# mederrata/spmf

Measured on AMD Instinct MI355X. Metric: elbo_steps_per_sec, higher is better.
Workload: dtype f32

## Files before the change

spmf_amd/csrc/col_pass.hip:

```cpp
#include "common.h"
#include "kernels.h"

namespace spmf {

#ifndef COL_WIDE_WAVES
#define COL_WIDE_WAVES 4
#endif
#ifndef COL_GRP
#define COL_GRP 4
#endif

template <int KP>
__device__ __forceinline__ void pack_block(const double* __restrict__ dacc, float* __restrict__ tail,
                                           const double* __restrict__ det_slots) {
  if (det_slots) {
    constexpr int LEN = kDaccHead + KP;
    constexpr int SEG = 256 / (LEN <= 32 ? 32 : (LEN <= 64 ? 64 : 128));
    constexpr int W = 256 / SEG;
    __shared__ double seg_sum[SEG][W];
    const int i = threadIdx.x % W, g = threadIdx.x / W;
    const int nb = min(max((int)det_slots[0], 0), kDetMaxBlocks);
    const int per = (nb + SEG - 1) / SEG;
    double v = 0.0;
    if (i < LEN) {
      const double* sl = det_slots + kDetMeta + i;
      const int b1 = min(nb, (g + 1) * per);
      for (int b = g * per; b < b1; ++b) v += sl[(size_t)b * LEN];
    }
    seg_sum[g][i] = v;
    __syncthreads();
    if (threadIdx.x < LEN) {
      double t = 0.0;
#pragma unroll
      for (int s = 0; s < SEG; ++s) t += seg_sum[s][threadIdx.x];
      const float hi = (float)t;
      tail[2 * threadIdx.x] = hi;
      tail[2 * threadIdx.x + 1] = (float)(t - (double)hi);
    }
    return;
  }
  const int i = threadIdx.x;
  if (i < kDaccHead + KP) fold_dacc(i, dacc, tail, KP);
}

template <int KP, int LIK, int EPL, bool PACKED>
__global__ __launch_bounds__(256, EPL == 4 ? COL_WIDE_WAVES : 1) void col_pass_kernel(
    int D, int n_panels, int row_base, int blocks_per_panel,
    const int32_t* __restrict__ item_ptr, const int4* __restrict__ items,
    const int32_t* __restrict__ pc_row, const float* __restrict__ pc_val,
    const float* __restrict__ pc_gval, const float* __restrict__ Vp,
    const float* __restrict__ phi, const float* __restrict__ z, const float* __restrict__ gzs,
    float* __restrict__ gAp, float* __restrict__ gVp, float* __restrict__ gphi,
    const uint8_t* __restrict__ ctype, const int32_t* __restrict__ item_mid, int half_sel,
    int64_t Brows, int64_t acc_stride, const double* __restrict__ pack_dacc,
    float* __restrict__ pack_tail, int64_t dacc_stride, const uint32_t* __restrict__ pc_ent,
    int panel_rows, float* __restrict__ det_part, int64_t det_part_stride,
    const double* __restrict__ det_slots, int64_t det_stride) {
  static_assert(EPL == 1 || EPL == 4, "entries per lane and fetch: 1 or 4");
  static_assert(!PACKED || EPL == 4, "the packed lists are read by the wide fetch only");
  if (pack_dacc && blockIdx.x == 0) {
    pack_block<KP>(pack_dacc + (size_t)blockIdx.y * dacc_stride, pack_tail + (size_t)blockIdx.y * acc_stride,
                   det_slots ? det_slots + (size_t)blockIdx.y * det_stride : nullptr);
    return;
  }
  if (gridDim.y > 1) {
    const size_t sd = blockIdx.y;
    Vp += sd * (size_t)D * KP;
    phi += sd * (size_t)D;
    z += sd * (size_t)Brows * KP;
    gzs += sd * (size_t)Brows * KP;
    gAp += sd * (size_t)acc_stride;
    gVp += sd * (size_t)acc_stride;
    gphi += sd * (size_t)acc_stride;
  }
  constexpr int LPN = KP / 4;
  constexpr int NG = 64 / LPN;
  const GTable zt = gtable(z, Brows, KP), gt = gtable(gzs, Brows, KP);
  constexpr int GRP = EPL == 4 ? COL_GRP : (LPN < COL_GRP ? LPN : COL_GRP);
  static_assert((EPL * LPN) % GRP == 0, "a fetch is a whole number of gather groups");
  __shared__ __attribute__((aligned(16))) float stage[4][NG][2 * KP];
  const int lane = threadIdx.x & 63;
  const int sub = lane % LPN, grp = lane / LPN;
  const int bp_row = grp * LPN * 4;
  const int wid = threadIdx.x >> 6;
  const int64_t L = (int64_t)blockIdx.x - (pack_dacc ? 1 : 0);
  int p, ib;
  if (n_panels < 8) {
    p = (int)(L / blocks_per_panel);
    ib = (int)(L % blocks_per_panel);
  } else {
    const int x = (int)(L & 7);
    const int64_t q = L >> 3;
    p = 8 * (int)(q / blocks_per_panel) + x;
    ib = (int)(q % blocks_per_panel);
  }
  if (p >= n_panels) return;
  const int ilo = half_sel == 2 ? item_mid[p] : item_ptr[p];
  const int ihi = half_sel == 1 ? item_mid[p] : item_ptr[p + 1];
  const int i0 = ilo + ib * 4 * NG;
  if (i0 >= ihi) return;
  const int it = i0 + wid * NG + grp;
  const bool ok = it < ihi;
  int cur = 0, end = 0, d = 0;
  if (ok) {
    const int4 im = items[it];
    cur = im.x;
    end = im.x + im.y;
    d = im.z;
  }
  const float4 vp = ok ? gather4<LPN>(Vp, d, sub) : make_float4(0.f, 0.f, 0.f, 0.f);
  const float ph = ok ? phi[d] : 1.f;
  const bool bern = LIK == 2 || LIK == 4 || (LIK == 3 && ok && ctype[d]);
  float4 gV = make_float4(0.f, 0.f, 0.f, 0.f), gA = gV;
  float gph = 0.f;

  struct __attribute__((packed, aligned(4))) I4 { int x, y, z, w; };
  struct __attribute__((packed, aligned(4))) F4 { float x, y, z, w; };
  constexpr int FE = EPL * LPN;
  struct Raw {
    int r[EPL];
    float x[EPL], g[EPL];
    int cnt;
  };
  auto fetch_raw = [&](Raw& f) {
    f.cnt = min(FE, end - cur);
    const int e = cur + EPL * sub;
#pragma unroll
    for (int t = 0; t < EPL; ++t) {
      f.r[t] = 0;
      f.x[t] = 0.f;
      f.g[t] = 0.f;
    }
    if (EPL * sub < f.cnt) {
      if constexpr (EPL == 4) {
        if (PACKED) {
          const I4 w = *reinterpret_cast<const I4*>(reinterpret_cast<const int32_t*>(pc_ent) + e);
          f.r[0] = w.x; f.r[1] = w.y; f.r[2] = w.z; f.r[3] = w.w;
        } else {
          const I4 w = *reinterpret_cast<const I4*>(pc_row + e);
          const F4 v = *reinterpret_cast<const F4*>(pc_val + e);
          f.r[0] = w.x; f.r[1] = w.y; f.r[2] = w.z; f.r[3] = w.w;
          f.x[0] = v.x; f.x[1] = v.y; f.x[2] = v.z; f.x[3] = v.w;
        }
        if (LIK == 1 || LIK == 4) {
          const F4 v = *reinterpret_cast<const F4*>(pc_gval + e);
          f.g[0] = v.x; f.g[1] = v.y; f.g[2] = v.z; f.g[3] = v.w;
        }
      } else {
        f.r[0] = pc_row[e];
        f.x[0] = pc_val[e];
        if (LIK == 1 || LIK == 4) f.g[0] = pc_gval[e];
      }
    }
    cur += f.cnt;
  };
  const int pbase = PACKED ? p * panel_rows : -row_base;
  auto decode = [&](const Raw& f, int (&rr_)[EPL], float (&xx_)[EPL], float (&gx_)[EPL]) {
    const int left = f.cnt - EPL * sub;
#pragma unroll
    for (int t = 0; t < EPL; ++t) {
      const bool on = left > t;
      if (PACKED) {
        const uint32_t w = (uint32_t)f.r[t];
        rr_[t] = on ? (int)(w >> 16) + pbase : kPadRow;
        xx_[t] = on ? (float)(w & 0xffffu) : 0.f;
      } else {
        rr_[t] = on ? f.r[t] + pbase : kPadRow;
        xx_[t] = on ? f.x[t] : 0.f;
      }
      gx_[t] = on ? f.g[t] : 0.f;
    }
  };

  Raw fa, fb, fc;
  fetch_raw(fa);
  if (EPL == 1) fetch_raw(fb);
  while (__any(fa.cnt > 0)) {
    if (EPL == 1) fetch_raw(fc);
    else fetch_raw(fb);
    int rr0[EPL];
    float xx0[EPL], gx0[EPL];
    decode(fa, rr0, xx0, gx0);
    const int cnt0 = fa.cnt;
#pragma unroll
    for (int g0 = 0; g0 < FE; g0 += GRP) {
      if (__any(cnt0 > g0)) {
        float4 zz[GRP], gg[GRP];
        float xv[GRP], gv[GRP];
#pragma unroll
        for (int j = 0; j < GRP; ++j) {
          const int q = g0 + j;
          const int sa = bp_row + (q / EPL) * 4;
          const int b = __builtin_amdgcn_ds_bpermute(sa, rr0[q % EPL]);
          xv[j] = __int_as_float(__builtin_amdgcn_ds_bpermute(sa, __float_as_int(xx0[q % EPL])));
          gv[j] = (LIK == 1 || LIK == 4) ? __int_as_float(__builtin_amdgcn_ds_bpermute(sa, __float_as_int(gx0[q % EPL])))
                                         : xv[j];
          zz[j] = gather4<LPN>(zt, b, sub);
          gg[j] = gather4<LPN>(gt, b, sub);
        }
#pragma unroll
        for (int j = 0; j < GRP; ++j) {
          if (bern) {
            float wv = xv[j];
            if (LIK == 4) wv *= expf(fminf(group_sum<LPN>(dot4(zz[j], vp)), kYSat));
            gV = fma4(wv, zz[j], gV);
            gA = fma4(gv[j], gg[j], gA);
            gph += xv[j];
          } else {
            const float y = group_sum<LPN>(dot4(zz[j], vp));
            float ey = 1.f;
            const float r = (LIK == 1 ? expm1_dec(fminf(y, kYSat), ey) : y) + ph;
            const float xr = (r > 0.f && r < INFINITY) ? xv[j] * __builtin_amdgcn_rcpf(r)
                                                       : (xv[j] > 0.f ? 1.f : 0.f);
            gV = fma4(LIK == 1 ? xr * ey : xr, zz[j], gV);
            gA = fma4(gv[j], gg[j], gA);
            gph += xr;
          }
        }
      }
    }
    if (EPL == 1) {
      fa = fb;
      fb = fc;
    } else {
      fa = fb;
    }
  }
  if (det_part) {
    if (ok) {
      float4* dst = reinterpret_cast<float4*>(det_part + (size_t)blockIdx.y * det_part_stride +
                                              (size_t)(it - item_ptr[0]) * det_part_len(KP));
      dst[sub] = gV;
      dst[LPN + sub] = gA;
      if (sub == 0) dst[2 * LPN] = make_float4(gph, 0.f, 0.f, 0.f);
    }
    return;
  }
  float4* st4 = reinterpret_cast<float4*>(&stage[wid][grp][0]);
  st4[sub] = gV;
  st4[LPN + sub] = gA;
  __builtin_amdgcn_wave_barrier();
  const float* flat = &stage[wid][0][0];
#pragma unroll
  for (int i = 0; i < (NG * 2 * KP) / 64; ++i) {
    const int e = i * 64 + lane;
    const int c = e / (2 * KP), rem = e % (2 * KP);
    const int dd = __shfl(d, c * LPN);
    const int okc = __shfl((int)ok, c * LPN);
    const float v = flat[e];
    if (okc && v != 0.f) {
      float* dst = (rem >= KP ? gAp + (size_t)dd * KP + (rem - KP) : gVp + (size_t)dd * KP + rem);
      atomicAdd(dst, v);
    }
  }
  if (ok && sub == 0 && gph != 0.f) atomicAdd(&gphi[d], gph);
}

template <int KP>
static bool launch_col_t(const ColArgs& a, hipStream_t st) {
  constexpr int NG = 64 / (KP / 4);
  const int per_block = 4 * NG;
  const int bpp = (a.max_items_per_panel + per_block - 1) / per_block;
  if (bpp < 1) return false;
  const int64_t nt = (a.n_panels + 7) / 8;
  const int64_t nb = (a.n_panels < 8 ? (int64_t)a.n_panels * bpp : nt * bpp * 8) + (a.pack_dacc ? 1 : 0);
  const int4* items = reinterpret_cast<const int4*>(a.items);
#define SPMF_COL_ARGS                                                                            \
  dim3((unsigned)nb, a.S > 1 ? a.S : 1), dim3(256), 0, st, a.D, a.n_panels, a.row_base, bpp,   \
      a.item_ptr, items, a.pc_row, a.pc_val, a.pc_gval, a.Vp, a.phi, a.z, a.gzs, a.gAp, a.gVp, \
      a.gphi, a.ctype, a.item_mid, a.half_sel, a.B, a.acc_stride, a.pack_dacc, a.pack_tail,     \
      a.dacc_stride, a.pc_ent, a.panel_rows, a.det_part, a.det_part_stride, a.det_slots, a.det_stride
  const bool wide = a.pc_pad >= KP - 1;
  const bool packed = wide && a.pc_ent && a.panel_rows > 0 && a.panel_rows <= 65536;
#define SPMF_COL_LAUNCH(L_)                                                                        \
  do {                                                                                             \
    if (packed)                                                                                    \
      hipLaunchKernelGGL((col_pass_kernel<KP, L_, 4, true>), SPMF_COL_ARGS);                       \
    else if (wide)                                                                                 \
      hipLaunchKernelGGL((col_pass_kernel<KP, L_, 4, false>), SPMF_COL_ARGS);                      \
    else                                                                                           \
      hipLaunchKernelGGL((col_pass_kernel<KP, L_, 1, false>), SPMF_COL_ARGS);                      \
  } while (0)
  if (a.logt == 4) SPMF_COL_LAUNCH(4);
  else if (a.logt == 3) SPMF_COL_LAUNCH(3);
  else if (a.logt == 2) SPMF_COL_LAUNCH(2);
  else if (a.logt == 1) SPMF_COL_LAUNCH(1);
  else SPMF_COL_LAUNCH(0);
#undef SPMF_COL_LAUNCH
#undef SPMF_COL_ARGS
  return true;
}

template <int KP>
__global__ __launch_bounds__(256) void det_reduce_kernel(int D, int n_panels, const int32_t* __restrict__ list_first,
                                                         const int32_t* __restrict__ item_pos,
                                                         const int32_t* __restrict__ item_ptr,
                                                         const float* __restrict__ part, int64_t part_stride,
                                                         float* __restrict__ gAp, float* __restrict__ gVp,
                                                         float* __restrict__ gphi, int64_t acc_stride) {
  constexpr int LPN = KP / 4;
  const int sub = threadIdx.x % LPN;
  const int d = blockIdx.x * (256 / LPN) + threadIdx.x / LPN;
  if (d >= D) return;
  part += (size_t)blockIdx.y * part_stride;
  gAp += (size_t)blockIdx.y * acc_stride;
  gVp += (size_t)blockIdx.y * acc_stride;
  gphi += (size_t)blockIdx.y * acc_stride;
  const int it0 = item_ptr[0];
  float4 gV = make_float4(0.f, 0.f, 0.f, 0.f), gA = gV;
  float gph = 0.f;
  auto add_item = [&](int r) {
    const float4* src = reinterpret_cast<const float4*>(part + (size_t)(item_pos[r] - it0) * det_part_len(KP));
    const float4 a = src[sub], b = src[LPN + sub];
    gV.x += a.x; gV.y += a.y; gV.z += a.z; gV.w += a.w;
    gA.x += b.x; gA.y += b.y; gA.z += b.z; gA.w += b.w;
    if (sub == 0) gph += src[2 * LPN].x;
  };
  constexpr int DP = 8;
  for (int p0 = 0; p0 < n_panels; p0 += DP) {
    int r0[DP], r1[DP], jp[DP];
#pragma unroll
    for (int i = 0; i < DP; ++i) {
      const bool on = p0 + i < n_panels;
      const int32_t* lf = list_first + (size_t)(on ? p0 + i : p0) * D + d;
      r0[i] = on ? lf[0] : 0;
      r1[i] = on ? lf[1] : 0;
    }
#pragma unroll
    for (int i = 0; i < DP; ++i) jp[i] = r1[i] > r0[i] ? item_pos[r0[i]] - it0 : 0;
    float4 a[DP], b[DP];
    float g[DP];
#pragma unroll
    for (int i = 0; i < DP; ++i) {
      const float4* src = reinterpret_cast<const float4*>(part + (size_t)jp[i] * det_part_len(KP));
      const bool on = r1[i] > r0[i];
      a[i] = on ? src[sub] : make_float4(0.f, 0.f, 0.f, 0.f);
      b[i] = on ? src[LPN + sub] : make_float4(0.f, 0.f, 0.f, 0.f);
      g[i] = (on && sub == 0) ? src[2 * LPN].x : 0.f;
    }
#pragma unroll
    for (int i = 0; i < DP; ++i) {
      if (r1[i] > r0[i]) {
        gV.x += a[i].x; gV.y += a[i].y; gV.z += a[i].z; gV.w += a[i].w;
        gA.x += b[i].x; gA.y += b[i].y; gA.z += b[i].z; gA.w += b[i].w;
        if (sub == 0) gph += g[i];
        for (int r = r0[i] + 1; r < r1[i]; ++r) add_item(r);
      }
    }
  }
  reinterpret_cast<float4*>(gVp + (size_t)d * KP)[sub] = gV;
  reinterpret_cast<float4*>(gAp + (size_t)d * KP)[sub] = gA;
  if (sub == 0) gphi[d] = gph;
}

void launch_det_reduce(const DetReduceArgs& a, hipStream_t st) {
  if (a.D <= 0 || a.n_panels <= 0) return;
  with_kp<64>(a.KP, [&](auto kp) {
    constexpr int KP = decltype(kp)::value, cols = 256 / (KP / 4);
    hipLaunchKernelGGL((det_reduce_kernel<KP>), dim3((a.D + cols - 1) / cols, a.S > 1 ? a.S : 1), dim3(256), 0, st,
                       a.D, a.n_panels, a.list_first, a.item_pos, a.item_ptr, a.part, a.part_stride, a.gAp, a.gVp,
                       a.gphi, a.acc_stride);
  });
}

bool launch_col_pass(int KP, const ColArgs& a, hipStream_t st) {
  if (KP > 64) return launch_col_widek(KP, a, st);
  bool ok = false;
  return with_kp<64>(KP, [&](auto kp) { ok = launch_col_t<decltype(kp)::value>(a, st); }) && ok;
}

}
```

Baseline: 393.4.

## Add eight-entries-per-lane packed fetch path for small KP column pass

Adds an EPL=8 variant of the column pass kernel for packed entry lists when KP is at most 32 and padding allows, so each lane loads two 16-byte vectors per fetch and more gathers are in flight per list read. The main loop becomes a do-while that prefetches only while entries remain, which skips a useless final fetch. The cost is more registers per lane and a larger unrolled gather body, which may lower occupancy or spill.

```diff
diff --git a/spmf_amd/csrc/col_pass.hip b/spmf_amd/csrc/col_pass.hip
--- a/spmf_amd/csrc/col_pass.hip
+++ b/spmf_amd/csrc/col_pass.hip
@@ -9,6 +9,7 @@
 #ifndef COL_GRP
 #define COL_GRP 4
 #endif
+constexpr int kCol8MaxKP = 32;
 
 template <int KP>
 __device__ __forceinline__ void pack_block(const double* __restrict__ dacc, float* __restrict__ tail,
@@ -44,7 +45,7 @@
 }
 
 template <int KP, int LIK, int EPL, bool PACKED>
-__global__ __launch_bounds__(256, EPL == 4 ? COL_WIDE_WAVES : 1) void col_pass_kernel(
+__global__ __launch_bounds__(256, EPL >= 4 ? COL_WIDE_WAVES : 1) void col_pass_kernel(
     int D, int n_panels, int row_base, int blocks_per_panel,
     const int32_t* __restrict__ item_ptr, const int4* __restrict__ items,
     const int32_t* __restrict__ pc_row, const float* __restrict__ pc_val,
@@ -56,8 +57,9 @@
     float* __restrict__ pack_tail, int64_t dacc_stride, const uint32_t* __restrict__ pc_ent,
     int panel_rows, float* __restrict__ det_part, int64_t det_part_stride,
     const double* __restrict__ det_slots, int64_t det_stride) {
-  static_assert(EPL == 1 || EPL == 4, "entries per lane and fetch: 1 or 4");
-  static_assert(!PACKED || EPL == 4, "the packed lists are read by the wide fetch only");
+  static_assert(EPL == 1 || EPL == 4 || EPL == 8, "entries per lane and fetch: 1, 4 or 8");
+  static_assert(!PACKED || EPL >= 4, "the packed lists are read by the wide fetches only");
+  static_assert(EPL != 8 || PACKED, "eight entries per lane: the packed lists only");
   if (pack_dacc && blockIdx.x == 0) {
     pack_block<KP>(pack_dacc + (size_t)blockIdx.y * dacc_stride, pack_tail + (size_t)blockIdx.y * acc_stride,
                    det_slots ? det_slots + (size_t)blockIdx.y * det_stride : nullptr);
@@ -76,7 +78,7 @@
   constexpr int LPN = KP / 4;
   constexpr int NG = 64 / LPN;
   const GTable zt = gtable(z, Brows, KP), gt = gtable(gzs, Brows, KP);
-  constexpr int GRP = EPL == 4 ? COL_GRP : (LPN < COL_GRP ? LPN : COL_GRP);
+  constexpr int GRP = EPL >= 4 ? COL_GRP : (LPN < COL_GRP ? LPN : COL_GRP);
   static_assert((EPL * LPN) % GRP == 0, "a fetch is a whole number of gather groups");
   __shared__ __attribute__((aligned(16))) float stage[4][NG][2 * KP];
   const int lane = threadIdx.x & 63;
@@ -132,19 +134,22 @@
       f.g[t] = 0.f;
     }
     if (EPL * sub < f.cnt) {
-      if constexpr (EPL == 4) {
-        if (PACKED) {
-          const I4 w = *reinterpret_cast<const I4*>(reinterpret_cast<const int32_t*>(pc_ent) + e);
-          f.r[0] = w.x; f.r[1] = w.y; f.r[2] = w.z; f.r[3] = w.w;
-        } else {
-          const I4 w = *reinterpret_cast<const I4*>(pc_row + e);
-          const F4 v = *reinterpret_cast<const F4*>(pc_val + e);
-          f.r[0] = w.x; f.r[1] = w.y; f.r[2] = w.z; f.r[3] = w.w;
-          f.x[0] = v.x; f.x[1] = v.y; f.x[2] = v.z; f.x[3] = v.w;
-        }
-        if (LIK == 1 || LIK == 4) {
-          const F4 v = *reinterpret_cast<const F4*>(pc_gval + e);
-          f.g[0] = v.x; f.g[1] = v.y; f.g[2] = v.z; f.g[3] = v.w;
+      if constexpr (EPL >= 4) {
+#pragma unroll
+        for (int h = 0; h < EPL; h += 4) {
+          if (PACKED) {
+            const I4 w = *reinterpret_cast<const I4*>(reinterpret_cast<const int32_t*>(pc_ent) + e + h);
+            f.r[h] = w.x; f.r[h + 1] = w.y; f.r[h + 2] = w.z; f.r[h + 3] = w.w;
+          } else {
+            const I4 w = *reinterpret_cast<const I4*>(pc_row + e + h);
+            const F4 v = *reinterpret_cast<const F4*>(pc_val + e + h);
+            f.r[h] = w.x; f.r[h + 1] = w.y; f.r[h + 2] = w.z; f.r[h + 3] = w.w;
+            f.x[h] = v.x; f.x[h + 1] = v.y; f.x[h + 2] = v.z; f.x[h + 3] = v.w;
+          }
+          if (LIK == 1 || LIK == 4) {
+            const F4 v = *reinterpret_cast<const F4*>(pc_gval + e + h);
+            f.g[h] = v.x; f.g[h + 1] = v.y; f.g[h + 2] = v.z; f.g[h + 3] = v.w;
+          }
         }
       } else {
         f.r[0] = pc_row[e];
@@ -175,9 +180,10 @@
   Raw fa, fb, fc;
   fetch_raw(fa);
   if (EPL == 1) fetch_raw(fb);
-  while (__any(fa.cnt > 0)) {
-    if (EPL == 1) fetch_raw(fc);
-    else fetch_raw(fb);
+  bool more;
+  do {
+    more = EPL == 1 || __any(cur < end);
+    if (more) fetch_raw(EPL == 1 ? fc : fb);
     int rr0[EPL];
     float xx0[EPL], gx0[EPL];
     decode(fa, rr0, xx0, gx0);
@@ -222,10 +228,11 @@
     if (EPL == 1) {
       fa = fb;
       fb = fc;
-    } else {
+      more = __any(fa.cnt > 0);
+    } else if (more) {
       fa = fb;
     }
-  }
+  } while (more);
   if (det_part) {
     if (ok) {
       float4* dst = reinterpret_cast<float4*>(det_part + (size_t)blockIdx.y * det_part_stride +
@@ -272,11 +279,22 @@
       a.dacc_stride, a.pc_ent, a.panel_rows, a.det_part, a.det_part_stride, a.det_slots, a.det_stride
   const bool wide = a.pc_pad >= KP - 1;
   const bool packed = wide && a.pc_ent && a.panel_rows > 0 && a.panel_rows <= 65536;
+  constexpr bool has8 = KP <= kCol8MaxKP, has4 = !has8 || KP - 1 < 7;
 #define SPMF_COL_LAUNCH(L_)                                                                        \
   do {                                                                                             \
-    if (packed)                                                                                    \
-      hipLaunchKernelGGL((col_pass_kernel<KP, L_, 4, true>), SPMF_COL_ARGS);                       \
-    else if (wide)                                                                                 \
+    if constexpr (has8) {                                                                          \
+      if (packed && a.pc_pad >= 7) {                                                               \
+        hipLaunchKernelGGL((col_pass_kernel<KP, L_, 8, true>), SPMF_COL_ARGS);                     \
+        break;                                                                                     \
+      }                                                                                            \
+    }                                                                                              \
+    if constexpr (has4) {                                                                          \
+      if (packed) {                                                                                \
+        hipLaunchKernelGGL((col_pass_kernel<KP, L_, 4, true>), SPMF_COL_ARGS);                     \
+        break;                                                                                     \
+      }                                                                                            \
+    }                                                                                              \
+    if (wide)                                                                                      \
       hipLaunchKernelGGL((col_pass_kernel<KP, L_, 4, false>), SPMF_COL_ARGS);                      \
     else                                                                                           \
       hipLaunchKernelGGL((col_pass_kernel<KP, L_, 1, false>), SPMF_COL_ARGS);                      \
```

New measurement: 397.6, median of 6. 1.01x the previous value.
